# ChristianFeldmann/libHM

Measured on AMD Instinct MI355X. Metric: decoded Mpixels/s (luma), 2160p Main10 reconstruction + loop filters, higher is better.
Workload: dtype int16 samples / int32 accumulate; 1 GPU; 3840x2160 Main10 lowdelay_P pictures, pre-parsed CTU metadata: prep+MC+dequant/IT/recon+deblock+SAO, batch of 16 independent pictures per step, inputs resident in HBM; sub_benchmark=full, streams=2, parallelism=frame-parallel, 1 process per GPU, no data-path collective

## Files before the change

### libhm_amd/csrc/hmgpu_api.hip

```cpp
#include "hmgpu_dev.h"
#include "packed_format.h"

#include <algorithm>
#include <chrono>
#include <atomic>
#include <cstdio>
#include <cstring>
#include <cstdlib>
#include <cmath>
#include <map>
#include <memory>
#include <mutex>
#include <tuple>
#include <new>
#include <thread>
#include <unordered_map>
#include <vector>

using namespace hmgpu;

namespace {

enum { K_PREP = 0, K_MC_LUMA, K_MC_CHROMA, K_ITX, K_DBK_VER, K_DBK_HOR, K_SAO, K_EXTEND, K_H2D, K_INTRA, K_FILTER, K_UNPACK };
const char* const kKernelNames[HMGPU_NUM_KERNELS] = {"prep", "mc_luma", "mc_chroma", "itx", "deblock_ver", "deblock_hor", "sao",
// ... 367 lines not shown
  return HMGPU_OK;
}

hmgpu_status run_recon(hmgpu_ctx* c, const Batch& b, bool any_intra, bool any_wp, bool any_cells, bool any_bi, bool any_islice) {
  int max_ctus = 0;
  for (int i = 0; i < b.n; i++) max_ctus = std::max(max_ctus, b.num_ctus[i]);
  { ProfScope ps(c, K_PREP); launch_prep(c->d_pics, b, max_ctus, c->parts, any_intra, any_bi, any_cells || c->fmt != 1, c->fmt, c->stream); }
  if (c->fmt != 1) {
    for (int i = 0; i < b.n; i++) {
      const PicDev& d = c->pics[b.pic[i]].dev;
      HIP_TRY(c, hipMemsetAsync(d.resid[1], 0, (size_t)((char*)d.resid[2] - (char*)d.resid[1]) + c->coef_elems[2] * sizeof(int16_t), c->stream));
    }
  }
  McArgs ma;
  memset(&ma, 0, sizeof(ma));
  ma.n = b.n; ma.width = c->seq.width; ma.height = c->seq.height; ma.log2ctu = c->seq.log2_ctu_size; ma.ctus_w = c->ctus_w;
  ma.tw = c->grid_w / 2; ma.npics = c->seq.max_pictures;
  ma.slab = c->plane_slab; ma.pic_stride = 2 * c->plane_bytes; ma.slab_bytes = ma.pic_stride * c->pics.size(); ma.sao_off = (uint32_t)c->plane_bytes;
  for (size_t i = 0; i < c->pics.size(); i++)
    if (c->pics[i].sao_applied) (i < 32 ? ma.sao_mask_lo : ma.sao_mask_hi) |= 1u << (i & 31);
  for (int i = 0; i < b.n; i++) {
    const PicDev& d = c->pics[b.pic[i]].dev;
    ma.first_ctu[i] = b.first_ctu[i]; ma.num_ctus[i] = b.num_ctus[i];
    ma.tmv[i] = d.tmv; ma.slices[i] = d.slices;
  }
  const PicDev& d0 = c->pics[b.pic[0]].dev;
  const char* const base0 = (const char*)c->pics[b.pic[0]].planes;
  uint32_t bps = (uint32_t)std::max(4, std::min(b.n >= 4 ? 12 : 24, max_ctus / 8 + 1));
  {
    ItxArgs ia;
    memset(&ia, 0, sizeof(ia));
    ia.n = b.n; ia.class_mask = 0xf;
    for (int k = 0; k < 3; k++) { ia.rtw[k] = (c->grid_w / 2) >> (k ? c->csx : 0); ia.bd[k] = d0.bd[k]; }
    ia.csx = c->csx; ia.csy = c->csy;
    for (int k = 0; k < 4; k++) ia.tu_cap[k] = c->tu_cap[k];
    for (int i = 0; i < b.n; i++) {
      const PicDev& d = c->pics[b.pic[i]].dev;
      for (int k = 0; k < 4; k++) ia.tu[i][k] = d.tu[k];
      ia.tu_count[i] = d.tu_count;
      for (int k = 0; k < 3; k++) { ia.coef[i][k] = d.coef[k]; ia.resid[i][k] = d.resid[k]; }
      ia.sl_m[i] = d.sl_m;
    }
    ProfScope ps(c, K_ITX);
    launch_itx(ia, bps, c->stream);
    bool any_ccp = false;
    for (int i = 0; i < b.n; i++) any_ccp |= c->pics[b.pic[i]].dev.ccp[0] != nullptr;
    if (any_ccp) launch_ccp(c->d_pics, b, max_ctus, c->stream);
  }
  {
    ProfScope ps(c, K_MC_LUMA);
    ma.pitch = c->pitch[0]; ma.bd = c->seq.bit_depth_luma;
    ma.origin_off = (uint32_t)((const char*)d0.rec[0] - base0);
    ma.rtw = c->grid_w / 2;
    for (int i = 0; i < b.n; i++) { ma.dst[i] = c->pics[b.pic[i]].dev.rec[0]; ma.resid[i] = c->pics[b.pic[i]].dev.resid[0]; }
    launch_mc_luma(ma, max_ctus, any_wp, any_bi, c->stream);
    if (any_cells) launch_mc_luma_cells(c->d_pics, c->d_finals, b, max_ctus, c->seq.log2_ctu_size, any_wp, c->stream);
  }
  if (c->fmt != 1) {
    ProfScope ps(c, K_MC_CHROMA);
    launch_mc_chroma_fmt(c->d_pics, c->d_finals, b, max_ctus, c->seq.log2_ctu_size, c->fmt, any_wp, c->stream);
  } else if (c->seq.chroma_format != 0) {
    ProfScope ps(c, K_MC_CHROMA);
    ma.pitch = c->pitch[1]; ma.bd = c->seq.bit_depth_chroma;
    ma.origin_off = (uint32_t)((const char*)d0.rec[1] - base0);
    ma.cr_off = 0;
    ma.rtw = c->grid_w / 4;
    for (int i = 0; i < b.n; i++) {
      const PicDev& d = c->pics[b.pic[i]].dev;
      ma.dst[i] = d.rec[1]; ma.dst2[i] = d.rec[2]; ma.resid[i] = d.resid[1]; ma.resid2[i] = d.resid[2];
    }
    launch_mc_chroma(ma, max_ctus, any_wp, any_bi, c->stream);
    if (any_cells) launch_mc_chroma_cells(c->d_pics, c->d_finals, b, max_ctus, c->seq.log2_ctu_size, any_wp, c->stream);
  }
  if (any_intra) {
    ProfScope ps(c, K_INTRA);
    launch_intra(c->d_pics, b, c->d_ctu_order, c->num_ctus, !any_islice, c->stream);
    if (c->fmt == 2) launch_intra_chroma_422(c->d_pics, b, c->stream);
    for (int i = 0; i < b.n; i++) if (std::find(c->intra_launched.begin(), c->intra_launched.end(), b.pic[i]) == c->intra_launched.end()) c->intra_launched.push_back(b.pic[i]);
  }
  HIP_TRY(c, hipGetLastError());
  return HMGPU_OK;
}

hmgpu_status run_filter(hmgpu_ctx* c, const Batch& b, int stages) {
  bool all_sao = stages == 7 && c->fmt == 1;
  for (int i = 0; i < b.n && all_sao; i++) all_sao = c->pics[b.pic[i]].sao_any;
  if (all_sao) {
    bool nofilt = false;
    for (int i = 0; i < b.n; i++) nofilt |= c->pics[b.pic[i]].dev.any_nofilt != 0;
    { ProfScope ps(c, K_FILTER); launch_filter_fused(c->d_pics, b, c->seq.width, c->seq.height, nofilt, c->stream); }
    HIP_TRY(c, hipGetLastError());
    return HMGPU_OK;
  }
  if (stages & 1) { ProfScope ps(c, K_DBK_VER); launch_deblock(c->d_pics, b, 0, c->seq.width, c->seq.height, c->stream);
                    if (c->fmt != 1) launch_deblock_chroma_fmt(c->d_pics, b, 0, c->seq.width, c->seq.height, c->stream); }
  if (stages & 2) { ProfScope ps(c, K_DBK_HOR); launch_deblock(c->d_pics, b, 1, c->seq.width, c->seq.height, c->stream);
                    if (c->fmt != 1) launch_deblock_chroma_fmt(c->d_pics, b, 1, c->seq.width, c->seq.height, c->stream); }
  if (stages & 4) {
    bool any = false;
    for (int i = 0; i < b.n; i++) any |= c->pics[b.pic[i]].sao_any;
    if (any) { ProfScope ps(c, K_SAO); launch_sao(c->d_pics, b, c->seq.width, c->seq.height, c->csx, c->csy, c->stream); }
  }
  HIP_TRY(c, hipGetLastError());
  return HMGPU_OK;
}

hmgpu_status stage_sao(hmgpu_ctx* c, Picture& p, const hmgpu_pic_params* pp, const hmgpu_sao_param* sao,
                       const std::vector<uint16_t>& slice_idx, const std::vector<uint16_t>& tile_idx) {
  const int n = c->num_ctus;
  std::vector<const hmgpu_sao_param*> res((size_t)n * 3);
  std::vector<SaoDev>& dev = p.h_saoprm;
  dev.resize((size_t)n * 3);
  bool any = false;
  for (int a = 0; a < n; a++) {
    const int cx = a % c->ctus_w, cy = a / c->ctus_w;
    const hmgpu_sao_param* const* merge[2] = {nullptr, nullptr};
    auto same = [&](int o) { return slice_idx[o] == slice_idx[a] && tile_idx[o] == tile_idx[a]; };
    if (cx > 0 && same(a - 1)) merge[HMGPU_SAO_MERGE_LEFT] = &res[(size_t)(a - 1) * 3];
    if (cy > 0 && same(a - c->ctus_w)) merge[HMGPU_SAO_MERGE_ABOVE] = &res[(size_t)(a - c->ctus_w) * 3];
    unsigned avail = 1u << 4;
    for (int k = 0; k < 9; k++) {
      if (k == 4) continue;
      const int nx = cx + k % 3 - 1, ny = cy + k / 3 - 1;
      if (nx < 0 || nx >= c->ctus_w || ny < 0 || ny >= c->ctus_h) continue;
      const int o = ny * c->ctus_w + nx;
      bool ok = true;
      if (slice_idx[o] != slice_idx[a]) {
        const SliceDev& later = p.slices[std::max(slice_idx[o], slice_idx[a])];
        ok = later.lf_across_slices != 0;
      }
      if (ok && !pp->lf_across_tiles) ok = tile_idx[o] == tile_idx[a];
      if (ok) avail |= 1u << k;
    }
    for (int comp = 0; comp < 3; comp++) {
      const hmgpu_sao_param* r = &sao[(size_t)a * 3 + comp];
      if (r->mode_idc == HMGPU_SAO_MERGE) {
        if (r->type_idc < 0 || r->type_idc > 1 || !merge[r->type_idc]) return HMGPU_EINVAL;
        r = merge[r->type_idc][comp];
      }
      res[(size_t)a * 3 + comp] = r;
      const int shift = comp == 0 ? pp->sao_offset_shift_luma : pp->sao_offset_shift_chroma;
      SaoDev& d = dev[(size_t)a * 3 + comp];
      memset(&d, 0, sizeof(d));
      d.type = r->mode_idc == HMGPU_SAO_OFF ? -1 : (int8_t)r->type_idc;
      d.avail = (uint16_t)avail;
      if (d.type == HMGPU_SAO_BO) {
        d.band = (uint8_t)(r->type_aux_info & 31);
        for (int i = 0; i < 4; i++) d.off[i] = (int8_t)(r->offset[(r->type_aux_info + i) & 31] * (1 << shift));
      } else if (d.type >= 0) {
        for (int i = 0; i < 5; i++) d.off[i] = (int8_t)(r->offset[i] * (1 << shift));
      }
      any |= d.type >= 0;
    }
  }
  p.sao_any = any;
  HIP_TRY(c, h2d_small(c, p.dev.saoprm, dev.data(), dev.size() * sizeof(SaoDev), c->stream));
  return HMGPU_OK;
}

}

extern "C" {

const char* hmgpu_status_string(hmgpu_status s) {
  switch (s) {
    case HMGPU_OK: return "ok";
    case HMGPU_EINVAL: return "invalid argument";
    case HMGPU_EDEVICE: return "device (HIP) error";
    case HMGPU_EUNSUPPORTED: return "coding tool not supported";
    case HMGPU_ENOMEM: return "out of memory";
  }
  return "?";
}
const char* hmgpu_kernel_name(int32_t k) { return (k >= 0 && k < HMGPU_NUM_KERNELS) ? kKernelNames[k] : ""; }

int32_t hmgpu_num_ctus(const hmgpu_seq_params* seq) {
  const int c = 1 << seq->log2_ctu_size;
  return ((seq->width + c - 1) / c) * ((seq->height + c - 1) / c);
}
int32_t hmgpu_parts_per_ctu(const hmgpu_seq_params* seq) { return 1 << (2 * seq->log2_ctu_size - 4); }

hmgpu_status hmgpu_create(const hmgpu_seq_params* seq, int device_ordinal, hmgpu_ctx** out) {
  if (!seq || !out) return HMGPU_EINVAL;
  *out = nullptr;
  if (seq->width <= 0 || seq->height <= 0 || (seq->width & 7) || (seq->height & 7)) return HMGPU_EINVAL;
  if (seq->log2_ctu_size < 4 || seq->log2_ctu_size > 6) return HMGPU_EINVAL;
  if (seq->max_pictures < 1 || seq->max_pictures > kMaxPics) return HMGPU_EINVAL;
  if (seq->chroma_format < 0 || seq->chroma_format > 3) return HMGPU_EINVAL;
  if (seq->range_ext_flags & ~(HMGPU_REXT_ROTATION | HMGPU_REXT_IMPLICIT_RDPCM | HMGPU_REXT_EXPLICIT_RDPCM | HMGPU_REXT_INTRA_SMOOTHING_DISABLED)) return HMGPU_EUNSUPPORTED;
  if (seq->bit_depth_luma < 8 || seq->bit_depth_luma > 12 || seq->bit_depth_chroma < 8 || seq->bit_depth_chroma > 12) return HMGPU_EUNSUPPORTED;
  hmgpu_ctx* c = new (std::nothrow) hmgpu_ctx();
  if (!c) return HMGPU_ENOMEM;
  c->seq = *seq;
  c->device = device_ordinal;
  c->host_timing = getenv("HMGPU_HOST_TIMING") != nullptr;
  hipError_t e = hipSetDevice(device_ordinal);
  if (e == hipSuccess) e = hipStreamCreateWithFlags(&c->stream, hipStreamNonBlocking);
  if (e == hipSuccess) e = hipStreamCreateWithFlags(&c->stream2, hipStreamNonBlocking);
  if (e == hipSuccess) e = hipStreamCreateWithFlags(&c->copy_stream, hipStreamNonBlocking);
  if (e == hipSuccess) e = hipStreamCreateWithFlags(&c->copy_stream2, hipStreamNonBlocking);
  if (e == hipSuccess) e = hipEventCreateWithFlags(&c->copy_join, hipEventDisableTiming);
  if (e == hipSuccess) e = hipHostMalloc((void**)&c->bounce, hmgpu_ctx::kBounceSegs * hmgpu_ctx::kBounceSeg, hipHostMallocDefault);
  for (int g = 0; g < hmgpu_ctx::kBounceSegs && e == hipSuccess; g++)
    for (int k = 0; k < 3 && e == hipSuccess; k++) e = hipEventCreateWithFlags(&c->bounce_ev[g][k], hipEventDisableTiming);
  for (int k = 0; k < 8 && e == hipSuccess; k++) e = hipEventCreateWithFlags(&c->copy_ev[k], hipEventDisableTiming);
  for (int k = 0; k < 8 && e == hipSuccess; k++) e = hipEventCreateWithFlags(&c->use_ev[k], hipEventDisableTiming);
  for (int k = 0; k < 32 && e == hipSuccess; k++) e = hipEventCreateWithFlags(&c->dl_ev[k], hipEventDisableTiming | hipEventBlockingSync);
  if (e == hipSuccess) { e = hipHostMalloc((void**)&c->dl_fault, 32 * sizeof(uint32_t), hipHostMallocDefault); if (e == hipSuccess) memset(c->dl_fault, 0, 32 * sizeof(uint32_t)); }
  for (int k = 0; k < 2 && e == hipSuccess; k++) e = hipEventCreateWithFlags(&c->lane_ev[k], hipEventDisableTiming);
  if (e != hipSuccess) { delete c; return HMGPU_EDEVICE; }
  c->ctu = 1 << seq->log2_ctu_size; c->pw = c->ctu / 4; c->parts = c->pw * c->pw;
  c->ctus_w = (seq->width + c->ctu - 1) / c->ctu; c->ctus_h = (seq->height + c->ctu - 1) / c->ctu;
  c->num_ctus = c->ctus_w * c->ctus_h;
  c->grid_w = c->ctus_w * c->pw; c->grid_h = c->ctus_h * c->pw;
  c->fmt = seq->chroma_format == 0 ? 1 : seq->chroma_format;
  c->csx = c->fmt == 3 ? 0 : 1; c->csy = c->fmt == 1 ? 1 : 0;
  c->mx[0] = 128; c->mx[1] = c->mx[2] = 128 >> c->csx;
  c->my[0] = 80; c->my[1] = c->my[2] = 80 >> c->csy;
  c->pitch[0] = (int)align_up((size_t)seq->width, 64) + 2 * c->mx[0] + 64;
  c->pitch[1] = c->pitch[2] = kCStep * ((int)align_up((size_t)seq->width >> c->csx, 64) + 2 * c->mx[1] + 64);
  c->rows[0] = c->ctus_h * c->ctu + 2 * c->my[0] + 8; c->rows[1] = c->rows[2] = ((c->ctus_h * c->ctu) >> c->csy) + 2 * c->my[1] + 8;
  c->coef_elems[0] = (size_t)c->num_ctus * c->ctu * c->ctu;
  c->coef_elems[1] = c->coef_elems[2] = c->coef_elems[0] >> (c->csx + c->csy);
  {
    const size_t blocks = ((size_t)c->num_ctus * (c->parts / 4) + 255) / 256;
    const size_t per_shard = (blocks + kTuShards - 1) / kTuShards;
    const uint32_t per_block[4] = {4 * 384, 4 * 96, 4 * 24, 4 * 4};
    for (int k = 0; k < 4; k++) c->tu_cap[k] = (uint32_t)(per_shard * (c->fmt == 1 ? per_block[k] : 3u * (1024u >> (2 * k))));
  }
  c->pics.resize(seq->max_pictures);
  c->h_finals.resize(seq->max_pictures);
  hmgpu_status st = HMGPU_OK;
  c->plane_bytes = plane_set_bytes(c);
  if (hipMalloc((void**)&c->plane_slab, c->plane_bytes * 2 * seq->max_pictures) != hipSuccess ||
      hipMemset(c->plane_slab, 0, c->plane_bytes * 2 * seq->max_pictures) != hipSuccess) st = HMGPU_EDEVICE;
  for (int i = 0; i < seq->max_pictures && st == HMGPU_OK; i++) st = alloc_picture(c, c->pics[i]);
  if (st == HMGPU_OK) {
    {
      std::vector<int32_t> order;
      for (int d = 0; d <= 2 * (c->ctus_h - 1) + c->ctus_w - 1; d++)
        for (int r = 0; r < c->ctus_h; r++) { const int col = d - 2 * r; if (col >= 0 && col < c->ctus_w) order.push_back(r * c->ctus_w + col); }
      if (hipMalloc((void**)&c->d_ctu_order, order.size() * sizeof(int32_t)) != hipSuccess ||
          hipMemcpy(c->d_ctu_order, order.data(), order.size() * sizeof(int32_t), hipMemcpyHostToDevice) != hipSuccess) st = HMGPU_EDEVICE;
    }
    if (hipMalloc((void**)&c->d_pics, sizeof(PicDev) * seq->max_pictures) != hipSuccess ||
        hipMalloc((void**)&c->d_finals, sizeof(PlaneSet) * seq->max_pictures) != hipSuccess) st = HMGPU_EDEVICE;
  }
  if (st == HMGPU_OK) {
    for (int i = 0; i < seq->max_pictures && st == HMGPU_OK; i++) { st = push_picdev(c, i); if (st == HMGPU_OK) st = push_final(c, i); }
    if (st == HMGPU_OK && hipStreamSynchronize(c->stream) != hipSuccess) st = HMGPU_EDEVICE;
  }
  if (st != HMGPU_OK) { hmgpu_destroy(c); return st; }
  *out = c;
  return HMGPU_OK;
}

void hmgpu_destroy(hmgpu_ctx* c) {
  if (!c) return;
  hipSetDevice(c->device);
  if (c->stream) hipStreamSynchronize(c->stream);
  prof_drain(c);
  for (EventPair& ep : c->free_events) { hipEventDestroy(ep.a); hipEventDestroy(ep.b); }
  if (c->host_timing && c->host_calls)
    fprintf(stderr, "hmgpu host time per hmgpu_decompress_pictures + hmgpu_filter_pictures (%llu calls): validate %.3f ms, slices %.3f, stage_inputs %.3f, recon launches %.3f, sao staging %.3f, filter launches %.3f\n",
            (unsigned long long)c->host_calls, 1e3 * c->host_s[0] / c->host_calls, 1e3 * c->host_s[1] / c->host_calls, 1e3 * c->host_s[2] / c->host_calls,
            1e3 * c->host_s[3] / c->host_calls, 1e3 * c->host_s[4] / c->host_calls, 1e3 * c->host_s[5] / c->host_calls);
  for (Picture& p : c->pics) free_picture(p);
  if (c->d_pics) hipFree(c->d_pics);
  if (c->d_finals) hipFree(c->d_finals);
  if (c->plane_slab) hipFree(c->plane_slab);
  if (c->scratch) hipFree(c->scratch);
  if (c->d_ctu_order) hipFree(c->d_ctu_order);
  if (c->stream) hipStreamDestroy(c->stream);
  if (c->stream2) hipStreamDestroy(c->stream2);
  if (c->copy_stream2) { hipStreamSynchronize(c->copy_stream2); hipStreamDestroy(c->copy_stream2); }
  if (c->copy_stream) { hipStreamSynchronize(c->copy_stream); hipStreamDestroy(c->copy_stream); }
  if (c->copy_join) hipEventDestroy(c->copy_join);
  for (int g = 0; g < hmgpu_ctx::kBounceSegs; g++) for (int k = 0; k < 3; k++) if (c->bounce_ev[g][k]) hipEventDestroy(c->bounce_ev[g][k]);
  if (c->bounce) (void)hipHostFree(c->bounce);
  for (int k = 0; k < 8; k++) { if (c->copy_ev[k]) hipEventDestroy(c->copy_ev[k]); if (c->use_ev[k]) hipEventDestroy(c->use_ev[k]); }
  for (hmgpu_staging* st : c->shared_stagings) {
    st->sharers.erase(std::remove(st->sharers.begin(), st->sharers.end(), c), st->sharers.end());
    if (st->reader == c) { st->reader = nullptr; st->copy_seq = 0; }
  }
  for (hmgpu_staging* st : c->stagings) {
    for (hmgpu_ctx* o : st->sharers) o->shared_stagings.erase(std::remove(o->shared_stagings.begin(), o->shared_stagings.end(), st), o->shared_stagings.end());
    if (st->host) hipHostFree(st->host);
    delete st;
  }
  for (int k = 0; k < 32; k++) if (c->dl_ev[k]) hipEventDestroy(c->dl_ev[k]);
  if (c->dl_fault) (void)hipHostFree(c->dl_fault);
  for (int k = 0; k < hmgpu_ctx::kHashStreams; k++) if (c->hash_stream[k]) { (void)hipStreamSynchronize(c->hash_stream[k]); (void)hipStreamDestroy(c->hash_stream[k]); }
  for (int k = 0; k < hmgpu_ctx::kHashSlots; k++) {
    if (c->hash_packed[k]) hipEventDestroy(c->hash_packed[k]);
    if (c->hash_done[k]) hipEventDestroy(c->hash_done[k]);
    if (c->hash_buf[k]) (void)hipFree(c->hash_buf[k]);
  }
  if (c->hash_dev) (void)hipFree(c->hash_dev);
  for (int k = 0; k < 2; k++) if (c->xfer_ev[k]) hipEventDestroy(c->xfer_ev[k]);
  for (int k = 0; k < 2; k++) if (c->exp_ev[k]) hipEventDestroy(c->exp_ev[k]);
  for (auto& sl : c->scale_slot) {
// ... 1389 lines not shown
  std::vector<std::vector<int>> all(n);
  {
    ProfScope ps(c, K_H2D);
    for (int i = 0; i < n && st == HMGPU_OK; i++) {
      const hmgpu_packed_job& j = jobs[i];
      Picture& p = c->pics[j.pic];
      const hipStream_t hs = (i & 1) ? c->copy_stream2 : c->copy_stream;
      wait_for_last_use(c, p, hs);
      if (p.sao_applied) { p.sao_applied = false; p.dev.sao_applied = 0; for (int k = 0; k < 3; k++) c->h_finals[j.pic].p[k] = p.dev.rec[k];
                           HIP_TRY(c, h2d_small(c, c->d_finals + j.pic, &c->h_finals[j.pic], sizeof(PlaneSet), hs)); }
      bool wp = false;
      { HostTimer ts(c, 1);
      for (int k = 0; k < j.num_slices && st == HMGPU_OK; k++) {
        st = register_slice(c, j.pic, k, j.slices[k], hs);
        all[i].push_back(k);
        wp |= j.slices[k] && j.slices[k]->weighted_pred != 0;
      }
      }
      SliceCall call;
      HostTimer ti(c, 2);
      if (st == HMGPU_OK) st = stage_packed(c, j, sums[i], all[i], wp, hs, &call);
      if (st != HMGPU_OK) break;
      b.pic[i] = j.pic; b.first_ctu[i] = 0; b.num_ctus[i] = c->num_ctus;
      ua.pic[i] = j.pic; ua.blob[i] = (const char*)p.blob;
      any_intra |= call.intra; any_wp |= call.wp; any_cells |= call.cells; any_bi |= call.bi; any_islice |= call.islice;
    }
    if (n > 1) {
      (void)hipEventRecord(c->copy_join, c->copy_stream2);
      (void)hipStreamWaitEvent(c->copy_stream, c->copy_join, 0);
    }
    if (st != HMGPU_OK) return st;
    c->copy_seq++;
    if (c->copy_seq > 8 && hipEventQuery(c->copy_ev[(c->copy_seq - 7) % 8]) == hipSuccess)
      for (auto it = c->packed_reads.begin(); it != c->packed_reads.end();) it = it->second <= c->copy_seq - 7 ? c->packed_reads.erase(it) : std::next(it);
    for (int i = 0; i < n; i++) c->packed_reads[jobs[i].blob] = c->copy_seq;
    HIP_TRY(c, hipEventRecord(c->copy_ev[c->copy_seq % 8], c->copy_stream));
    HIP_TRY(c, hipStreamWaitEvent(c->stream, c->copy_ev[c->copy_seq % 8], 0));
  }
  HostTimer tr(c, 3);
  { ProfScope ps(c, K_UNPACK); launch_unpack_input(c->d_pics, ua, c->num_ctus, c->stream); }
  HIP_TRY(c, hipGetLastError());
  for (int i = 0; i < n && st == HMGPU_OK; i++) st = extend_refs_of(c, jobs[i].pic, all[i]);
  if (st == HMGPU_OK) st = run_recon(c, b, any_intra, any_wp, any_cells, any_bi, any_islice);
  mark_use(c, b);
  return st;
}

hmgpu_status hmgpu_packed_wait(hmgpu_ctx* c, const void* blob) {
  if (!c || !blob) return HMGPU_EINVAL;
  const auto it = c->packed_reads.find(blob);
  if (it == c->packed_reads.end()) return HMGPU_OK;
  hipSetDevice(c->device);
  const uint64_t seq = c->copy_seq - it->second < 8 ? it->second : c->copy_seq;
  if (hipEventSynchronize(c->copy_ev[seq % 8]) != hipSuccess) return HMGPU_EDEVICE;
  return HMGPU_OK;
}

hmgpu_status hmgpu_filter_pictures(hmgpu_ctx* c, int32_t n, const hmgpu_filter_job* jobs) {
  if (!c || !jobs || n < 1 || n > kMaxBatch) return HMGPU_EINVAL;
  for (int i = 0; i < n; i++) {
    if (!valid_pic(c, jobs[i].pic) || !jobs[i].pp) return HMGPU_EINVAL;
    if (jobs[i].pp->sao_enabled && !jobs[i].sao) return HMGPU_EINVAL;
    for (int k = 0; k < i; k++) if (jobs[k].pic == jobs[i].pic) return HMGPU_EINVAL;
  }
  hipSetDevice(c->device);
  Batch b; memset(&b, 0, sizeof(b));
  b.n = n;
  { HostTimer tsao(c, 4);
  for (int i = 0; i < n; i++) {
    Picture& p = c->pics[jobs[i].pic];
    p.sao_any = false;
    if (jobs[i].pp->sao_enabled) {
      std::vector<uint16_t> sidx = p.h_slice_idx, tidx = p.h_tile_idx;
      sidx.resize(c->num_ctus, 0);
      tidx.resize(c->num_ctus, 0);
      hmgpu_status st = stage_sao(c, p, jobs[i].pp, jobs[i].sao, sidx, tidx);
      if (st != HMGPU_OK) return st;
    }
    p.filter_ready = true;
    b.pic[i] = jobs[i].pic; b.first_ctu[i] = 0; b.num_ctus[i] = c->num_ctus;
  }
  }
  HostTimer tf(c, 5);
  hmgpu_status st = run_filter(c, b, 7);
  if (st != HMGPU_OK) return st;
  for (int i = 0; i < n && st == HMGPU_OK; i++) {
    Picture& p = c->pics[jobs[i].pic];
    if (p.sao_any) {
      p.sao_applied = true; p.dev.sao_applied = 1;
      st = push_final(c, jobs[i].pic);
      if (st == HMGPU_OK) st = push_picdev(c, jobs[i].pic);
    }
    p.extended = true;
  }
  if (st != HMGPU_OK) return st;
  { ProfScope ps(c, K_EXTEND); launch_extend(c->d_pics, b, c->seq.width, c->seq.height, c->mx[0], c->my[0], c->csx, c->csy, c->stream); }
  HIP_TRY(c, hipGetLastError());
  mark_use(c, b);
  return HMGPU_OK;
}

hmgpu_status hmgpu_filter_picture_stages(hmgpu_ctx* c, hmgpu_pic cur, const hmgpu_pic_params* pp, const hmgpu_sao_param* sao,
                                         int32_t stages) {
  if (!c || !valid_pic(c, cur) || !pp) return HMGPU_EINVAL;
  if ((stages & 4) && pp->sao_enabled && !sao) return HMGPU_EINVAL;
  hipSetDevice(c->device);
  Picture& p = c->pics[cur];
  p.sao_any = false;
  if ((stages & 4) && pp->sao_enabled) {
    std::vector<uint16_t> sidx = p.h_slice_idx, tidx = p.h_tile_idx;
    sidx.resize(c->num_ctus, 0);
    tidx.resize(c->num_ctus, 0);
    hmgpu_status st = stage_sao(c, p, pp, sao, sidx, tidx);
    if (st != HMGPU_OK) return st;
  }
  p.filter_ready = true;
  Batch b; memset(&b, 0, sizeof(b));
  b.n = 1; b.pic[0] = cur; b.first_ctu[0] = 0; b.num_ctus[0] = c->num_ctus;
  hmgpu_status st = run_filter(c, b, stages);
  if (st != HMGPU_OK) return st;
  if ((stages & 4) && p.sao_any) {
    p.sao_applied = true; p.dev.sao_applied = 1;
    st = push_final(c, cur);
    if (st == HMGPU_OK) st = push_picdev(c, cur);
    if (st != HMGPU_OK) return st;
  }
  p.extended = false;
  st = ensure_extended(c, cur);
  commit_use(c);
  return st;
}

hmgpu_status hmgpu_filter_picture(hmgpu_ctx* c, hmgpu_pic cur, const hmgpu_pic_params* pp, const hmgpu_sao_param* sao) {
  return hmgpu_filter_picture_stages(c, cur, pp, sao, 7);
}

hmgpu_status hmgpu_replay_batch(hmgpu_ctx* c, const hmgpu_pic* pics, int32_t n, int32_t stages, int32_t iters) {
  if (!c || !pics || n < 1 || n > kMaxBatch || iters < 0) return HMGPU_EINVAL;
  size_t ncalls = 0;
  for (int i = 0; i < n; i++) {
    if (!valid_pic(c, pics[i])) return HMGPU_EINVAL;
    if (i == 0) ncalls = c->pics[pics[i]].calls.size();
    else if (c->pics[pics[i]].calls.size() != ncalls) return HMGPU_EINVAL;
  }
  if ((stages & 8) && ncalls == 0) return HMGPU_EINVAL;
  hipSetDevice(c->device);
  const int lanes = (c->replay_streams == 2 && n >= 2 && !c->profiling) ? 2 : 1;
  hipStream_t const main_stream = c->stream;
  if (lanes == 2) {
    HIP_TRY(c, hipEventRecord(c->lane_ev[0], main_stream));
    HIP_TRY(c, hipStreamWaitEvent(c->stream2, c->lane_ev[0], 0));
  }
  hmgpu_status result = HMGPU_OK;
  for (int it = 0; it < iters && result == HMGPU_OK; it++) {
    for (int lane = 0; lane < lanes && result == HMGPU_OK; lane++) {
      const int lo = lanes == 2 ? (lane == 0 ? 0 : n / 2) : 0, hi = lanes == 2 ? (lane == 0 ? n / 2 : n) : n;
      c->stream = lane == 0 ? main_stream : c->stream2;
      if (stages & 8) {
        for (size_t k = 0; k < ncalls && result == HMGPU_OK; k++) {
          Batch b; memset(&b, 0, sizeof(b));
          b.n = hi - lo;
          bool any_intra = false, any_wp = false, any_cells = false, any_bi = false, any_islice = false;
          for (int i = lo; i < hi; i++) {
            const SliceCall& sc = c->pics[pics[i]].calls[k];
            b.pic[i - lo] = pics[i]; b.first_ctu[i - lo] = sc.first_ctu; b.num_ctus[i - lo] = sc.num_ctus;
            any_intra |= sc.intra; any_wp |= sc.wp; any_cells |= sc.cells; any_bi |= sc.bi; any_islice |= sc.islice;
          }
          result = ensure_refs_extended(c, b, k);
          if (result == HMGPU_OK) result = run_recon(c, b, any_intra, any_wp, any_cells, any_bi, any_islice);
        }
      }
      if ((stages & 7) && result == HMGPU_OK) {
        Batch b; memset(&b, 0, sizeof(b));
        b.n = hi - lo;
        for (int i = lo; i < hi; i++) { b.pic[i - lo] = pics[i]; b.first_ctu[i - lo] = 0; b.num_ctus[i - lo] = c->num_ctus; }
        result = run_filter(c, b, stages & 7);
        if (result == HMGPU_OK) {
          { ProfScope ps(c, K_EXTEND); launch_extend(c->d_pics, b, c->seq.width, c->seq.height, c->mx[0], c->my[0], c->csx, c->csy, c->stream); }
          if (hipGetLastError() != hipSuccess) result = HMGPU_EDEVICE;
        }
      }
    }
  }
  c->stream = main_stream;
  if (lanes == 2) {
    HIP_TRY(c, hipEventRecord(c->lane_ev[1], c->stream2));
    HIP_TRY(c, hipStreamWaitEvent(main_stream, c->lane_ev[1], 0));
  }
  for (int i = 0; i < n; i++) touch(c, pics[i]);
  commit_use(c);
  return result;
}

hmgpu_status hmgpu_set_streams(hmgpu_ctx* c, int32_t n) {
  if (!c || n < 1 || n > 2) return HMGPU_EINVAL;
  c->replay_streams = n;
  return HMGPU_OK;
}

hmgpu_status hmgpu_replay(hmgpu_ctx* c, hmgpu_pic cur, int32_t stages, int32_t iters) { return hmgpu_replay_batch(c, &cur, 1, stages, iters); }

hmgpu_status hmgpu_set_profiling(hmgpu_ctx* c, int32_t enable) {
  if (!c) return HMGPU_EINVAL;
  HIP_TRY(c, hipStreamSynchronize(c->stream));
  prof_drain(c);
  c->profiling = enable != 0;
  return HMGPU_OK;
}

hmgpu_status hmgpu_get_stats(hmgpu_ctx* c, hmgpu_stats* out, int32_t reset) {
  if (!c || !out) return HMGPU_EINVAL;
  HIP_TRY(c, hipStreamSynchronize(c->stream));
  prof_drain(c);
  memset(out, 0, sizeof(*out));
  for (int k = 0; k < HMGPU_NUM_KERNELS; k++) { out->kernel_ms[k] = c->kernel_ms[k]; out->kernel_launches[k] = c->kernel_launches[k]; }
  for (Picture& p : c->pics) {
    if (!p.in_use) continue;
    unsigned long long st[2 * kTuShards];
    HIP_TRY(c, hipMemcpy(st, p.dev.stats, sizeof(st), hipMemcpyDeviceToHost));
    for (int s = 0; s < kTuShards; s++) { out->intra_partitions += st[s]; out->inter_partitions += st[kTuShards + s]; }
    if (reset) HIP_TRY(c, hipMemset(p.dev.stats, 0, sizeof(st)));
  }
  if (reset) for (int k = 0; k < HMGPU_NUM_KERNELS; k++) { c->kernel_ms[k] = 0; c->kernel_launches[k] = 0; }
  return HMGPU_OK;
}

hmgpu_status hmgpu_inverse_transform_batch(hmgpu_ctx* c, int32_t log2_size, int32_t bit_depth, int32_t n, const int16_t* levels,
                                           const int8_t* qp_per, const int8_t* qp_rem, const uint8_t* flags, int16_t* resid) {
  if (!c || log2_size < 2 || log2_size > 5 || n < 1 || !levels || !qp_per || !qp_rem || !flags || !resid) return HMGPU_EINVAL;
  if (bit_depth < 8 || bit_depth > 12) return HMGPU_EUNSUPPORTED;
  hipSetDevice(c->device);
  const size_t elems = (size_t)n << (2 * log2_size);
  int16_t *d_lev = nullptr, *d_res = nullptr; int8_t *d_per = nullptr, *d_rem = nullptr; uint8_t* d_fl = nullptr;
  hmgpu_status st = HMGPU_OK;
  auto fail = [&](hipError_t e) { if (e != hipSuccess && st == HMGPU_OK) { c->last_err = (int32_t)e; st = HMGPU_EDEVICE; } };
  fail(hipMalloc((void**)&d_lev, elems * 2)); fail(hipMalloc((void**)&d_res, elems * 2));
  fail(hipMalloc((void**)&d_per, n)); fail(hipMalloc((void**)&d_rem, n)); fail(hipMalloc((void**)&d_fl, n));
  if (st == HMGPU_OK) {
    fail(hipMemcpy(d_lev, levels, elems * 2, hipMemcpyHostToDevice));
    fail(hipMemcpy(d_per, qp_per, n, hipMemcpyHostToDevice)); fail(hipMemcpy(d_rem, qp_rem, n, hipMemcpyHostToDevice));
    fail(hipMemcpy(d_fl, flags, n, hipMemcpyHostToDevice));
  }
  if (st == HMGPU_OK) {
    launch_itx_flat(log2_size, bit_depth, n, d_lev, d_per, d_rem, d_fl, d_res, c->stream);
    fail(hipGetLastError());
    fail(hipStreamSynchronize(c->stream));
    fail(hipMemcpy(resid, d_res, elems * 2, hipMemcpyDeviceToHost));
  }
  hipFree(d_lev); hipFree(d_res); hipFree(d_per); hipFree(d_rem); hipFree(d_fl);
  return st;
}

hmgpu_status hmgpu_mc_batch(hmgpu_ctx* c, int32_t is_chroma, int32_t bit_depth, const int16_t* ref_plane, int32_t ref_stride,
                            int32_t ref_w, int32_t ref_h, int32_t n, const int32_t* blocks, int32_t bi, int16_t* dst) {
  if (!c || !ref_plane || !blocks || !dst || n < 1 || ref_w < 1 || ref_h < 1 || ref_stride < ref_w) return HMGPU_EINVAL;
  if (bit_depth < 8 || bit_depth > 12) return HMGPU_EUNSUPPORTED;
  hipSetDevice(c->device);
  std::vector<int32_t> off(n);
  size_t total = 0;
  for (int i = 0; i < n; i++) {
// ... 40 lines not shown
```

### libhm_amd/csrc/hmgpu_dev.h

```cpp
#pragma once
#include <hip/hip_runtime.h>
#include <stdint.h>
#include "../../include/hmgpu.h"

namespace hmgpu {

constexpr int kMaxBatch = 16;
constexpr int kMaxPics = 64;
constexpr int kTuShards = 8;
constexpr int kCStep = 2;

struct __attribute__((aligned(16))) BlkInfo {
  int16_t mv[2][2];
  int8_t  ref[2];
  int8_t  qp;
  uint8_t flags;
  uint8_t edge;
  uint8_t log2cu;
  uint16_t slice;
};
static_assert(sizeof(BlkInfo) == 16, "BlkInfo must be 16 bytes");

enum : uint8_t {
  BF_VALID = 1,
  BF_INTRA = 2,
  BF_CBFY = 4,
  BF_MC_L0 = 8,
  BF_MC_L1 = 16,
  BF_NOFILT = 32,
};
enum : uint8_t {
  BE_VER_FILTER = 1,
  BE_VER_TRANSFORM = 2,
  BE_HOR_FILTER = 4,
  BE_HOR_TRANSFORM = 8,
};

struct __attribute__((aligned(8))) EdgeRec { uint16_t v[2], h[2]; };
static_assert(sizeof(EdgeRec) == 8, "EdgeRec must be 8 bytes");
__host__ __device__ constexpr uint32_t edge_unit_pack(int bs, int qp, bool p_nf, bool q_nf) {
  return (uint32_t)bs | ((uint32_t)(qp + 32) << 2) | ((p_nf ? 1u : 0u) << 9) | ((q_nf ? 1u : 0u) << 10);
}

struct __attribute__((aligned(16))) TileMv {
  int16_t ix0, iy0, ix1, iy1;
  uint8_t frac;
  uint8_t ref0, ref1;
  uint8_t flags;
  uint8_t ridx;
  uint8_t rmask;
  uint16_t slice;
};
static_assert(sizeof(TileMv) == 16, "TileMv must be 16 bytes");
enum : uint8_t { TM_ACTIVE = 1, TM_BI = 2, TM_FIRST_L1 = 4 };
__host__ __device__ constexpr int resid_slot(int row) { return ((row & 1) << 2) | ((row & 7) >> 1); }
enum : uint8_t { TR_LUMA = 15, TR_CB = 16, TR_CR = 32 };

struct TuRec {
  uint16_t x4, y4;
  uint8_t  comp_flags;
  int8_t   per, rem;
  uint8_t  xflags;
  uint32_t coef_off;
};
static_assert(sizeof(TuRec) == 12, "TuRec must be 12 bytes");

struct SliceDev {
  int32_t slice_type;
  int32_t cb_qp_offset, cr_qp_offset;
  int32_t pps_cb_qp_offset, pps_cr_qp_offset;
  int32_t deblocking_disable, beta_offset_div2, tc_offset_div2, lf_across_slices;
  int32_t ref_poc[2][HMGPU_MAX_REF];
  int8_t  ref_pic[2][HMGPU_MAX_REF];
  int32_t constrained_intra_pred;
  int32_t weighted_pred;
  int32_t wp_log2_denom[2];
  int16_t wp_weight[2][HMGPU_MAX_REF][3];
  int16_t wp_offset[2][HMGPU_MAX_REF][3];
};

struct SaoDev {
  int8_t  type;
  uint8_t band;
  uint16_t avail;
  int8_t  off[8];
};
static_assert(sizeof(SaoDev) == 12, "SaoDev layout");

struct PlaneSet { int16_t* p[3]; };

struct PicDev {
  int32_t width, height;
  int32_t bd[3];
// ... 200 lines not shown
```

### libhm_amd/csrc/k_filter.hip

```cpp
#include "hmgpu_dev.h"
#include "filter_core.h"
#include <type_traits>

namespace hmgpu {

namespace {
constexpr int kTW = 64, kTH = 64;
constexpr int kYC = kTW + 16, kYH = kTH + 8;
constexpr int kCC = kTW / 2 + 16, kCH = kTH / 2 + 4;
constexpr int kYW = kYC + 8, kCW = kCC + 8;

constexpr int kUnits = 9 * 18;
struct FilterLds {
  __attribute__((aligned(16))) int16_t y[kYH][kYW];
  __attribute__((aligned(16))) int16_t c[2][kCH][kCW];
  uint32_t unit[2][3][64];
  int32_t units[2][4];
};

struct SaoPrm { uint32_t w0, off_lo, off_hi; };
__device__ inline SaoPrm sao_fetch(const PicDev& P, int comp, int x, int row) {
  const int log2ctb = P.log2ctu - (comp ? 1 : 0);
  const int w = P.width >> (comp ? 1 : 0), h = P.height >> (comp ? 1 : 0);
  SaoPrm r = {0xffu, 0u, 0u};
  if (x < w && row < h) {
    const uint32_t* pw = reinterpret_cast<const uint32_t*>(P.saoprm + ((size_t)(row >> log2ctb) * P.ctus_w + (x >> log2ctb)) * 3 + comp);
    r.w0 = ldg(pw); r.off_lo = ldg(pw + 1); r.off_hi = ldg(pw + 2);
  }
  return r;
}

template <int W, bool NF>
__device__ inline u32x4 sao_group(const PicDev& P, int comp, const int16_t (*t)[W], int ox, int oy, int x, int row, const SaoPrm& prm) {
  const int cs = comp ? 1 : 0;
  const int w = P.width >> cs, h = P.height >> cs;
  const int log2ctb = P.log2ctu - cs;
  const int cx = x >> log2ctb, cy = row >> log2ctb;
  const uint32_t w0 = prm.w0;
  const int type = (int)(int8_t)(w0 & 0xff);
  const int16_t* line = &t[row - oy][x - ox];
  const u32x4 cur = *reinterpret_cast<const u32x4*>(line);
  if (type < 0) return cur;
  const uint32_t off_lo = prm.off_lo, off_hi = prm.off_hi;
  const int bd = P.bd[comp], maxv = (1 << bd) - 1;
  uint32_t out[4];
  if (type == HMGPU_SAO_BO) {
    const int shift = bd - 5, band0 = (w0 >> 8) & 0xff;
    const uint32_t c[4] = {cur.x, cur.y, cur.z, cur.w};
#pragma unroll
    for (int j = 0; j < 4; j++) {
      const uint32_t lo = c[j] & 0xffffu, hi = c[j] >> 16;
      const uint32_t k0 = min(((lo >> shift) - band0) & 31u, 4u), k1 = min(((hi >> shift) - band0) & 31u, 4u);
      const s16x2 off = lut_offsets(k0 | (k1 << 16), off_lo, 0u);
      out[j] = as_u32(__builtin_elementwise_min(__builtin_elementwise_max(as_s16x2(c[j]) + off, splat(0)), splat(maxv)));
    }
  } else {
    const int ctb = 1 << log2ctb;
    const int x0 = cx << log2ctb, y0 = cy << log2ctb;
    const int x1 = min(x0 + ctb, w) - 1, y1 = min(y0 + ctb, h) - 1;
    const unsigned av = w0 >> 16;
    auto run = [&](auto dxc, auto dyc) {
      constexpr int DX = decltype(dxc)::value, DY = decltype(dyc)::value;
      const int16_t* ra = line + DY * W;
      const int16_t* rb = line - DY * W;
      const u32x4 ea = *reinterpret_cast<const u32x4*>(ra), eb = *reinterpret_cast<const u32x4*>(rb);
      uint32_t na[4], nb[4];
      uint32_t la = 0, raa = 0, lb = 0, rbb = 0;
      if constexpr (DX < 0) { la = (uint16_t)ra[-1]; rbb = (uint16_t)rb[8]; }
      if constexpr (DX > 0) { raa = (uint16_t)ra[8]; lb = (uint16_t)rb[-1]; }
      shifted<DX>(ea, la, raa, na);
      shifted<-DX>(eb, lb, rbb, nb);
      sao_eo_core<DX, DY>(x, row, cur, na, nb, off_lo, off_hi, av, x0, y0, x1, y1, maxv, out);
    };
    switch (type) {
      case HMGPU_SAO_EO_0:   run(std::integral_constant<int, -1>{}, std::integral_constant<int, 0>{}); break;
      case HMGPU_SAO_EO_90:  run(std::integral_constant<int, 0>{}, std::integral_constant<int, -1>{}); break;
      case HMGPU_SAO_EO_135: run(std::integral_constant<int, -1>{}, std::integral_constant<int, -1>{}); break;
      default:               run(std::integral_constant<int, 1>{}, std::integral_constant<int, -1>{}); break;
    }
  }
  if (NF && P.any_nofilt) {
    uint32_t m[4];
    sao_exempt_mask(P, comp, x, row, m);
    const uint32_t c[4] = {cur.x, cur.y, cur.z, cur.w};
#pragma unroll
// ... 18 lines not shown
template <bool NF>
__device__ inline uint32_t edge_classify(const PicDev& P, uint32_t rec, int u, int x, int y) {
  if ((rec & 3u) == 0u) return 0u;
  const uint32_t bs = rec & 3u, qp = (rec >> 2) & 127u;
  const uint32_t p_nf = NF ? (rec >> 9) & 1u : 0u, q_nf = NF ? (rec >> 10) & 1u : 0u;
  const uint32_t slice = P.slice_idx ? (uint32_t)ldg(P.slice_idx + (size_t)(y >> P.log2ctu) * P.ctus_w + (x >> P.log2ctu)) : 0u;
  return (uint32_t)u | (bs << 8) | (p_nf << 10) | (q_nf << 11) | ((qp + 32u) << 12) | (slice << 20);
}

__device__ inline void push_units(uint32_t (&list)[3][64], int32_t (&count)[4], uint32_t rec, int t) {
  const unsigned long long m = __ballot(rec != 0u);
  const int wave = t >> 6, lane = t & 63;
  if (rec != 0u) list[wave][__popcll(m & ((1ull << lane) - 1ull))] = rec;
  if (lane == 0) count[wave] = __popcll(m);
}
__device__ inline uint32_t pop_unit(const uint32_t (&list)[3][64], const int32_t (&count)[4], int t) {
  const int c0 = count[0], c1 = count[1], c2 = count[2];
  if (t < c0) return list[0][t];
  if (t < c0 + c1) return list[1][t - c0];
  if (t < c0 + c1 + c2) return list[2][t - c0 - c1];
  return 0u;
}

template <int DIR, bool NF>
__device__ inline void edge_apply(const PicDev& P, FilterLds& L, int x0, int y0, uint32_t rec, const SliceLf& s0) {
  if (rec == 0u) return;
  const int u = rec & 0xff, bs = (rec >> 8) & 3, qp = (int)((rec >> 12) & 0xff) - 64, slice = rec >> 20;
  const bool p_nf = NF && ((rec >> 10) & 1), q_nf = NF && ((rec >> 11) & 1);
  const int x = DIR == 0 ? x0 + 8 * (u % 9) : x0 - 4 + 4 * (u % 18);
  const int y = DIR == 0 ? y0 - 4 + 4 * (u / 9) : y0 + 8 * (u / 18);
  const SliceLf sl = slice == 0 ? s0 : slice_lf(P.slices + slice);
  const int tc_off = sl.tc_off, beta_off = sl.beta_off;
  int16_t* base = &L.y[y - (y0 - 4)][x - (x0 - 8)];
  uint32_t a[8], b[8];
  if (DIR == 0) {
    uint32_t r[4][4];
#pragma unroll
    for (int i = 0; i < 4; i++) {
      const u32x2 lo = *reinterpret_cast<const u32x2*>(base + i * kYW - 4), hi = *reinterpret_cast<const u32x2*>(base + i * kYW);
      r[i][0] = lo.x; r[i][1] = lo.y; r[i][2] = hi.x; r[i][3] = hi.y;
    }
    rows_to_pairs(r[0], r[1], a);
    rows_to_pairs(r[2], r[3], b);
  } else {
#pragma unroll
    for (int k = 0; k < 8; k++) {
      const u32x2 v = *reinterpret_cast<const u32x2*>(base + (k - 4) * kYW);
      a[k] = v.x; b[k] = v.y;
    }
  }
  filter_luma_unit(a, b, bs, qp, tc_off, beta_off, P.bd[0], p_nf, q_nf);
  if (DIR == 0) {
    uint32_t r[4][4];
    pairs_to_rows(a, r[0], r[1]);
    pairs_to_rows(b, r[2], r[3]);
#pragma unroll
    for (int i = 0; i < 4; i++) {
      *reinterpret_cast<u32x2*>(base + i * kYW - 4) = (u32x2){r[i][0], r[i][1]};
      *reinterpret_cast<u32x2*>(base + i * kYW) = (u32x2){r[i][2], r[i][3]};
    }
  } else {
#pragma unroll
    for (int k = 1; k < 7; k++) *reinterpret_cast<u32x2*>(base + (k - 4) * kYW) = (u32x2){a[k], b[k]};
  }
  if (bs == 2 && ((DIR == 0 ? x : y) & 15) == 0 && !P.mono) {
    const int maxc = (1 << P.bd[1]) - 1;
#pragma unroll
    for (int comp = 1; comp < 3; comp++) {
      const int tc = chroma_tc(qp, comp == 1 ? sl.cb_off : sl.cr_off, tc_off, P.bd[comp]);
      int16_t* cb = &L.c[comp - 1][(y >> 1) - ((y0 >> 1) - 2)][(x >> 1) - ((x0 >> 1) - 8)];
#pragma unroll
      for (int i = 0; i < 2; i++) {
        int16_t* s = DIR == 0 ? cb + i * kCW : cb + i;
        const int o = DIR == 0 ? 1 : kCW;
        const int m2 = (uint16_t)s[-2 * o], m3 = (uint16_t)s[-o], m4 = (uint16_t)s[0], m5 = (uint16_t)s[o];
        const int delta = clip3(-tc, tc, ((((m4 - m3) << 2) + m2 - m5 + 4) >> 3));
        if (!p_nf) s[-o] = (int16_t)clip3(0, maxc, m3 + delta);
        if (!q_nf) s[0] = (int16_t)clip3(0, maxc, m4 - delta);
      }
    }
  }
}

}

template <bool NF>
__global__ void __launch_bounds__(256) k_filter_fused(const PicDev* __restrict__ pics, Batch b, int tiles_x, int tiles) {
  __shared__ FilterLds L;
  int slot, lb;
  if (!xcd_remap(blockIdx.x, b.n, tiles, slot, lb)) return;
  const PicDev& P = pics[b.pic[slot]];
  const int x0 = (lb % tiles_x) * kTW, y0 = (lb / tiles_x) * kTH;
  const int t = threadIdx.x;
  const int vx = x0 + 8 * (t % 9), vy = y0 - 4 + 4 * (t / 9), hx = x0 - 4 + 4 * (t % 18), hy = y0 + 8 * (t / 18);
  const uint32_t ev = edge_fetch<0>(P, vx, vy, t < kUnits), eh = edge_fetch<1>(P, hx, hy, t < kUnits);
  const SliceLf s0 = slice_lf(P.slices);
  int lx[2], ly[2];
  SaoPrm sl[2];
#pragma unroll
  for (int k = 0; k < 2; k++) {
    const int g = t + 256 * k;
    lx[k] = x0 + (g & 7) * 8; ly[k] = y0 + (g >> 3);
    sl[k] = sao_fetch(P, 0, lx[k], ly[k]);
  }
  const int ccomp = 1 + (t & 1), ccx = (x0 >> 1) + ((t >> 1) & 3) * 8, ccy = (y0 >> 1) + (t >> 3);
  const SaoPrm sc = sao_fetch(P, ccomp, ccx, ccy);
  constexpr int VPR = kYC / 8, VPC = kCC / 8, NY = (kYH * VPR + 255) / 256, NC = (2 * kCH * VPC + 255) / 256;
  u32x4 ty[NY], tc[NC];
  {
    const int16_t* src = P.rec[0] + (ptrdiff_t)(y0 - 4) * P.pitch[0] + (x0 - 8);
#pragma unroll
    for (int k = 0; k < NY; k++) {
      const int i = t + 256 * k, r = i / VPR, v = i % VPR;
      if (i < kYH * VPR) ty[k] = ldg4(src + (ptrdiff_t)r * P.pitch[0] + 8 * v);
    }
#pragma unroll
    for (int k = 0; k < NC; k++) {
      const int i = t + 256 * k, r = i / (2 * VPC), v = i % (2 * VPC);
      if (i < 2 * kCH * VPC) tc[k] = ldg4(P.rec[1] + (ptrdiff_t)((y0 >> 1) - 2 + r) * P.pitch[1] + kCStep * (((x0 >> 1) - 8) + 4 * v));
    }
  }
  if (t < 192) {
    push_units(L.unit[0], L.units[0], edge_classify<NF>(P, ev, t, vx, vy), t);
    push_units(L.unit[1], L.units[1], edge_classify<NF>(P, eh, t, hx, hy), t);
  }
#pragma unroll
  for (int k = 0; k < NY; k++) {
    const int i = t + 256 * k, r = i / VPR, v = i % VPR;
    if (i < kYH * VPR) *reinterpret_cast<u32x4*>(&L.y[r][8 * v]) = ty[k];
  }
#pragma unroll
  for (int k = 0; k < NC; k++) {
    const int i = t + 256 * k, r = i / (2 * VPC), v = i % (2 * VPC);
    if (i < 2 * kCH * VPC) {
      *reinterpret_cast<u32x2*>(&L.c[0][r][4 * v]) = u32x2{__builtin_amdgcn_perm(tc[k].y, tc[k].x, 0x05040100u), __builtin_amdgcn_perm(tc[k].w, tc[k].z, 0x05040100u)};
      *reinterpret_cast<u32x2*>(&L.c[1][r][4 * v]) = u32x2{__builtin_amdgcn_perm(tc[k].y, tc[k].x, 0x07060302u), __builtin_amdgcn_perm(tc[k].w, tc[k].z, 0x07060302u)};
    }
  }
  __syncthreads();
  edge_apply<0, NF>(P, L, x0, y0, pop_unit(L.unit[0], L.units[0], t), s0);
  __syncthreads();
  edge_apply<1, NF>(P, L, x0, y0, pop_unit(L.unit[1], L.units[1], t), s0);
  __syncthreads();
#pragma unroll
  for (int k = 0; k < 2; k++)
    if (lx[k] < P.width && ly[k] < P.height)
      stg4(P.sao[0] + (size_t)ly[k] * P.pitch[0] + lx[k], sao_group<kYW, NF>(P, 0, L.y, x0 - 8, y0 - 4, lx[k], ly[k], sl[k]));
  if (ccx < (P.width >> 1) && ccy < (P.height >> 1)) {
    const u32x4 own = sao_group<kCW, NF>(P, ccomp, L.c[ccomp - 1], (x0 >> 1) - 8, (y0 >> 1) - 2, ccx, ccy, sc);
    const bool odd = t & 1;
    const uint32_t r0 = (uint32_t)__shfl_xor((int)(odd ? own.x : own.z), 1, 64), r1 = (uint32_t)__shfl_xor((int)(odd ? own.y : own.w), 1, 64);
    const uint32_t cb0 = odd ? r0 : own.x, cb1 = odd ? r1 : own.y, cr0 = odd ? own.z : r0, cr1 = odd ? own.w : r1;
    const u32x4 o = {__builtin_amdgcn_perm(cr0, cb0, 0x05040100u), __builtin_amdgcn_perm(cr0, cb0, 0x07060302u),
                     __builtin_amdgcn_perm(cr1, cb1, 0x05040100u), __builtin_amdgcn_perm(cr1, cb1, 0x07060302u)};
    stg4(P.sao[1] + (size_t)ccy * P.pitch[1] + kCStep * (ccx + (odd ? 4 : 0)), o);
  }
}

void launch_filter_fused(const PicDev* pics, const Batch& b, int width, int height, bool nofilt, hipStream_t s) {
  const int tiles_x = (width + kTW - 1) / kTW, tiles = tiles_x * ((height + kTH - 1) / kTH);
  dim3 grid((unsigned)xcd_grid(b.n, tiles));
  if (nofilt) hipLaunchKernelGGL(k_filter_fused<true>, grid, dim3(256), 0, s, pics, b, tiles_x, tiles);
  else hipLaunchKernelGGL(k_filter_fused<false>, grid, dim3(256), 0, s, pics, b, tiles_x, tiles);
}

}
```

Baseline: 178,900 Mpixels/s.

## Fuse picture border extension into the fused filter kernel and skip launch_extend

Boundary tiles of the fused deblock+SAO kernel now stage their edge rows and columns in LDS that overlays the edge-unit lists. They then write the padding margins directly, so the separate extend kernel launch is skipped when the fused path runs. This removes one full kernel pass and its re-read of the picture borders. In exchange, boundary blocks take an extra barrier and more stores. The change also depends on the margins matching compile-time constants, and on correct corner handling for both luma and interleaved chroma.

```diff
diff --git a/libhm_amd/csrc/hmgpu_api.hip b/libhm_amd/csrc/hmgpu_api.hip
--- a/libhm_amd/csrc/hmgpu_api.hip
+++ b/libhm_amd/csrc/hmgpu_api.hip
@@ -473,14 +473,17 @@
   return HMGPU_OK;
 }
 
-hmgpu_status run_filter(hmgpu_ctx* c, const Batch& b, int stages) {
+hmgpu_status run_filter(hmgpu_ctx* c, const Batch& b, int stages, bool* margins) {
+  *margins = false;
   bool all_sao = stages == 7 && c->fmt == 1;
+  all_sao = all_sao && c->mx[0] == kMarginX && c->my[0] == kMarginY;
   for (int i = 0; i < b.n && all_sao; i++) all_sao = c->pics[b.pic[i]].sao_any;
   if (all_sao) {
     bool nofilt = false;
     for (int i = 0; i < b.n; i++) nofilt |= c->pics[b.pic[i]].dev.any_nofilt != 0;
     { ProfScope ps(c, K_FILTER); launch_filter_fused(c->d_pics, b, c->seq.width, c->seq.height, nofilt, c->stream); }
     HIP_TRY(c, hipGetLastError());
+    *margins = true;
     return HMGPU_OK;
   }
   if (stages & 1) { ProfScope ps(c, K_DBK_VER); launch_deblock(c->d_pics, b, 0, c->seq.width, c->seq.height, c->stream);
@@ -606,8 +609,8 @@
   c->grid_w = c->ctus_w * c->pw; c->grid_h = c->ctus_h * c->pw;
   c->fmt = seq->chroma_format == 0 ? 1 : seq->chroma_format;
   c->csx = c->fmt == 3 ? 0 : 1; c->csy = c->fmt == 1 ? 1 : 0;
-  c->mx[0] = 128; c->mx[1] = c->mx[2] = 128 >> c->csx;
-  c->my[0] = 80; c->my[1] = c->my[2] = 80 >> c->csy;
+  c->mx[0] = kMarginX; c->mx[1] = c->mx[2] = kMarginX >> c->csx;
+  c->my[0] = kMarginY; c->my[1] = c->my[2] = kMarginY >> c->csy;
   c->pitch[0] = (int)align_up((size_t)seq->width, 64) + 2 * c->mx[0] + 64;
   c->pitch[1] = c->pitch[2] = kCStep * ((int)align_up((size_t)seq->width >> c->csx, 64) + 2 * c->mx[1] + 64);
   c->rows[0] = c->ctus_h * c->ctu + 2 * c->my[0] + 8; c->rows[1] = c->rows[2] = ((c->ctus_h * c->ctu) >> c->csy) + 2 * c->my[1] + 8;
@@ -2163,7 +2166,8 @@
   }
   }
   HostTimer tf(c, 5);
-  hmgpu_status st = run_filter(c, b, 7);
+  bool margins;
+  hmgpu_status st = run_filter(c, b, 7, &margins);
   if (st != HMGPU_OK) return st;
   for (int i = 0; i < n && st == HMGPU_OK; i++) {
     Picture& p = c->pics[jobs[i].pic];
@@ -2175,7 +2179,7 @@
     p.extended = true;
   }
   if (st != HMGPU_OK) return st;
-  { ProfScope ps(c, K_EXTEND); launch_extend(c->d_pics, b, c->seq.width, c->seq.height, c->mx[0], c->my[0], c->csx, c->csy, c->stream); }
+  if (!margins) { ProfScope ps(c, K_EXTEND); launch_extend(c->d_pics, b, c->seq.width, c->seq.height, c->mx[0], c->my[0], c->csx, c->csy, c->stream); }
   HIP_TRY(c, hipGetLastError());
   mark_use(c, b);
   return HMGPU_OK;
@@ -2198,7 +2202,8 @@
   p.filter_ready = true;
   Batch b; memset(&b, 0, sizeof(b));
   b.n = 1; b.pic[0] = cur; b.first_ctu[0] = 0; b.num_ctus[0] = c->num_ctus;
-  hmgpu_status st = run_filter(c, b, stages);
+  bool margins;
+  hmgpu_status st = run_filter(c, b, stages, &margins);
   if (st != HMGPU_OK) return st;
   if ((stages & 4) && p.sao_any) {
     p.sao_applied = true; p.dev.sao_applied = 1;
@@ -2206,7 +2211,7 @@
     if (st == HMGPU_OK) st = push_picdev(c, cur);
     if (st != HMGPU_OK) return st;
   }
-  p.extended = false;
+  p.extended = margins;
   st = ensure_extended(c, cur);
   commit_use(c);
   return st;
@@ -2255,8 +2260,9 @@
         Batch b; memset(&b, 0, sizeof(b));
         b.n = hi - lo;
         for (int i = lo; i < hi; i++) { b.pic[i - lo] = pics[i]; b.first_ctu[i - lo] = 0; b.num_ctus[i - lo] = c->num_ctus; }
-        result = run_filter(c, b, stages & 7);
-        if (result == HMGPU_OK) {
+        bool margins = false;
+        result = run_filter(c, b, stages & 7, &margins);
+        if (result == HMGPU_OK && !margins) {
           { ProfScope ps(c, K_EXTEND); launch_extend(c->d_pics, b, c->seq.width, c->seq.height, c->mx[0], c->my[0], c->csx, c->csy, c->stream); }
           if (hipGetLastError() != hipSuccess) result = HMGPU_EDEVICE;
         }
diff --git a/libhm_amd/csrc/hmgpu_dev.h b/libhm_amd/csrc/hmgpu_dev.h
--- a/libhm_amd/csrc/hmgpu_dev.h
+++ b/libhm_amd/csrc/hmgpu_dev.h
@@ -9,6 +9,7 @@
 constexpr int kMaxPics = 64;
 constexpr int kTuShards = 8;
 constexpr int kCStep = 2;
+constexpr int kMarginX = 128, kMarginY = 80;
 
 struct __attribute__((aligned(16))) BlkInfo {
   int16_t mv[2][2];
diff --git a/libhm_amd/csrc/k_filter.hip b/libhm_amd/csrc/k_filter.hip
--- a/libhm_amd/csrc/k_filter.hip
+++ b/libhm_amd/csrc/k_filter.hip
@@ -1,6 +1,7 @@
 #include "hmgpu_dev.h"
 #include "filter_core.h"
 #include <type_traits>
+#include <cstddef>
 
 namespace hmgpu {
 
@@ -185,6 +186,38 @@
   }
 }
 
+struct MarginLds {
+  u32x4 row[2][2][kTW / 8];
+  uint32_t col[2][2][kTH];
+};
+static_assert(sizeof(MarginLds) <= sizeof(FilterLds::unit), "the margin staging must fit the edge-unit lists it overlays");
+static_assert(offsetof(FilterLds, unit) % 16 == 0, "MarginLds::row is accessed as 16-byte vectors");
+enum : unsigned { kSideLeft = 1, kSideRight = 2, kSideTop = 4, kSideBottom = 8 };
+static_assert(kMarginX % 8 == 0 && 256 % (kMarginX / 8) == 0 && (kMarginX / 8 & (kMarginX / 8 - 1)) == 0 && kMarginY % 2 == 0,
+              "write_margins: 16-byte vectors, a power-of-two number of lanes per band row");
+
+__device__ inline void write_margins(int16_t* pl, int pitch, int w16, int h, int x0, int y0, int th, int my, unsigned side,
+                                     const u32x4 (&row)[2][kTW / 8], const uint32_t (&col)[2][kTH], int t) {
+  const int nrows = min(th, h - y0), nv = min(kTW, w16 - x0) >> 3;
+  const int ra = (side & kSideTop) ? -my : 0, rb = nrows + ((side & kSideBottom) ? my : 0);
+#pragma unroll
+  for (int s = 0; s < 2; s++) {
+    if (!(side & (kSideLeft << s))) continue;
+    int16_t* dst = pl + (ptrdiff_t)y0 * pitch + (s ? w16 : -kMarginX) + 8 * (t & (kMarginX / 8 - 1));
+    for (int r = ra + t / (kMarginX / 8); r < rb; r += 256 / (kMarginX / 8)) {
+      const uint32_t v = col[s][clip3(0, nrows - 1, r)];
+      stg4(dst + (ptrdiff_t)r * pitch, u32x4{v, v, v, v});
+    }
+  }
+#pragma unroll
+  for (int s = 0; s < 2; s++) {
+    if (!(side & (kSideTop << s)) || (t & 7) >= nv) continue;
+    const u32x4 v = row[s][t & 7];
+    int16_t* dst = pl + (ptrdiff_t)(s ? h : -my) * pitch + x0 + 8 * (t & 7);
+    for (int r = t >> 3; r < my; r += 32) stg4(dst + (ptrdiff_t)r * pitch, v);
+  }
+}
+
 }
 
 template <bool NF>
@@ -245,18 +278,45 @@
   __syncthreads();
   edge_apply<1, NF>(P, L, x0, y0, pop_unit(L.unit[1], L.units[1], t), s0);
   __syncthreads();
+  const unsigned side = (x0 == 0 ? kSideLeft : 0u) | (x0 + kTW >= P.width ? kSideRight : 0u) | (y0 == 0 ? kSideTop : 0u) | (y0 + kTH >= P.height ? kSideBottom : 0u);
+  MarginLds& M = *reinterpret_cast<MarginLds*>(&L.unit[0][0][0]);
 #pragma unroll
   for (int k = 0; k < 2; k++)
-    if (lx[k] < P.width && ly[k] < P.height)
-      stg4(P.sao[0] + (size_t)ly[k] * P.pitch[0] + lx[k], sao_group<kYW, NF>(P, 0, L.y, x0 - 8, y0 - 4, lx[k], ly[k], sl[k]));
-  if (ccx < (P.width >> 1) && ccy < (P.height >> 1)) {
+    if (lx[k] < P.width && ly[k] < P.height) {
+      const u32x4 o = sao_group<kYW, NF>(P, 0, L.y, x0 - 8, y0 - 4, lx[k], ly[k], sl[k]);
+      stg4(P.sao[0] + (size_t)ly[k] * P.pitch[0] + lx[k], o);
+      if (side) {
+        const int gx = (lx[k] - x0) >> 3, gr = ly[k] - y0;
+        if ((side & kSideLeft) && gx == 0) M.col[0][0][gr] = (o.x & 0xffffu) * 0x10001u;
+        if (lx[k] + 8 == P.width) M.col[0][1][gr] = (o.w >> 16) * 0x10001u;
+        if (ly[k] == 0) M.row[0][0][gx] = o;
+        if (ly[k] == P.height - 1) M.row[0][1][gx] = o;
+      }
+    }
+  const int cw = P.width >> 1, ch = P.height >> 1;
+  if (ccx < cw && ccy < ch) {
     const u32x4 own = sao_group<kCW, NF>(P, ccomp, L.c[ccomp - 1], (x0 >> 1) - 8, (y0 >> 1) - 2, ccx, ccy, sc);
     const bool odd = t & 1;
     const uint32_t r0 = (uint32_t)__shfl_xor((int)(odd ? own.x : own.z), 1, 64), r1 = (uint32_t)__shfl_xor((int)(odd ? own.y : own.w), 1, 64);
     const uint32_t cb0 = odd ? r0 : own.x, cb1 = odd ? r1 : own.y, cr0 = odd ? own.z : r0, cr1 = odd ? own.w : r1;
     const u32x4 o = {__builtin_amdgcn_perm(cr0, cb0, 0x05040100u), __builtin_amdgcn_perm(cr0, cb0, 0x07060302u),
                      __builtin_amdgcn_perm(cr1, cb1, 0x05040100u), __builtin_amdgcn_perm(cr1, cb1, 0x07060302u)};
-    stg4(P.sao[1] + (size_t)ccy * P.pitch[1] + kCStep * (ccx + (odd ? 4 : 0)), o);
+    const int px = ccx + (odd ? 4 : 0);
+    if (px < cw) {
+      stg4(P.sao[1] + (size_t)ccy * P.pitch[1] + kCStep * px, o);
+      if (side) {
+        const int gr = ccy - (y0 >> 1);
+        if ((side & kSideLeft) && px == 0) M.col[1][0][gr] = o.x;
+        if (px + 4 == cw) M.col[1][1][gr] = o.w;
+        if (ccy == 0) M.row[1][0][t & 7] = o;
+        if (ccy == ch - 1) M.row[1][1][t & 7] = o;
+      }
+    }
+  }
+  if (side) {
+    __syncthreads();
+    write_margins(P.sao[0], P.pitch[0], P.width, P.height, x0, y0, kTH, kMarginY, side, M.row[0], M.col[0], t);
+    write_margins(P.sao[1], P.pitch[1], P.width, ch, x0, y0 >> 1, kTH / 2, kMarginY / 2, side, M.row[1], M.col[1], t);
   }
 }
 
```

New measurement: 181,700 Mpixels/s, median of 6. 1.6% higher.
